# Hengle/AkariRender-1

Measured on AMD Instinct MI355X. Metric: Msamples/sec (whole node), 10M-tri scene 1080p 1024spp, 1/2/4/8 MI355X, higher is better.
Workload: dtype f32; 1 GPU; C3 synthetic triangle soup (SURVEY.md §8d); triangles=10000002, width=1920, height=1080, spp=1025, max_depth=5, tile=64, parallelism=tile-split x1, bvh_leaf=4, builder=sbvh, form=k_path, ordered_fetch=True

## Files before the change

akarirender-1_amd/csrc/capi.hip:

```cpp
#include <hip/hip_runtime.h>

#include <algorithm>
#include <atomic>
#include <chrono>
#include <cmath>
#include <cstring>
#include <map>
#include <memory>
#include <stdexcept>
#include <string>
#include <thread>
#include <vector>

#include "akr_device.h"
#include "bvh_build.h"
#include "kernels.h"
#include "options.h"
#include "path_plan.h"

using namespace akr;

#define HIPCHK(x)                                                                                        \
    do {                                                                                                 \
        hipError_t e_ = (x);                                                                             \
        if (e_ != hipSuccess) throw std::runtime_error(std::string(#x) + " failed: " + hipGetErrorString(e_)); \
    } while (0)

namespace {

template <class T>
struct DBuf {
    T *p = nullptr;
    size_t n = 0;
    DBuf() = default;
    DBuf(const DBuf &) = delete;
    DBuf &operator=(const DBuf &) = delete;
    ~DBuf() { release(); }
    void release() {
        if (p) (void)hipFree(p);
        p = nullptr;
        n = 0;
    }
    void reserve(size_t count) {
        if (count <= n && p) return;
        release();
        size_t c = std::max<size_t>(count, 1);
        HIPCHK(hipMalloc(reinterpret_cast<void **>(&p), c * sizeof(T)));
        n = c;
    }
    void upload(const T *h, size_t count, hipStream_t st) {
// ... 91 lines not shown
    std::string err;
    Options opt;
    hipEvent_t ev_done = nullptr;
    bool done_recorded = false;
    DBuf<uint32_t> d_bad;
    uint32_t *h_check = nullptr, *d_check_host = nullptr;
    uint32_t *h_fault = nullptr, *d_fault_host = nullptr;
    DBuf<uint4> d_probe;
    uint64_t probe_n = 0;
    bool probe_ok = false;

    std::vector<float> verts;
    std::vector<int32_t> idx;
    std::vector<float> normals, texcoords;
    std::vector<int32_t> matid;
    std::vector<uint32_t> mesh_base{0};
    std::vector<akr_texture> texs;
    std::vector<akr_material> mats;
    std::vector<float> images;
    std::vector<int64_t> img_off;
    std::vector<int32_t> img_w, img_h;
    std::vector<akr_area_light> lights;
    std::vector<float> power;
    bool scene_dirty = true;
    bool accel_built = false;
    akr_accel_info info{};
    BvhOutput bvh;
    Bvh4Output bvh4;

    DBuf<akr_bvh_node> d_nodes;
    DBuf<akr_bvh4_node> d_wnodes;
    DBuf<float4> d_wleaves;
    uint32_t wide_root_dev = AKR_CHILD_EMPTY;
    uint64_t bvh_dev_bytes = 0;
    DBuf<float4> d_tris;
    DBuf<ShadeTri> d_shade_tri;
    DBuf<float> d_tc, d_images, d_cdf, d_func;
    DBuf<MatDev> d_mats;
    DBuf<TexDev> d_texs;
    DBuf<LightDev> d_lights;
    DBuf<uint32_t> d_mesh_base;
    float func_int = 0;
    int32_t n_lights = 0;
    int32_t n_mats = 0;
    bool has_image_tex = false;
    bool simple_shading = true;

    CameraDev cam{};
    bool cam_set = false;

    EnvDev env{};
    DBuf<float4> d_env_map;
    DBuf<float> d_env_tab;
    bool env_on() const { return env.n > 0; }
    const EnvDev &require_env() const {
        if (!env_on()) throw std::runtime_error("no environment light (akr_hip_upload_environment)");
        return env;
    }

    size_t cap = 0;
    std::vector<uint4> h_tiles;
    uint64_t n_pix_last = 0;
    DBuf<uint4> d_tiles;
    struct Session {
        bool valid = false, seeded = false;
        uint64_t n = 0;
// ... 494 lines not shown
        HIPCHK(hipMemsetAsync(d_owork.p, 0, kTraceWords * sizeof(uint32_t), ms));
        const uint32_t sub = (uint32_t)opt.path_order_sub, n_rays = (uint32_t)(((uint64_t)N + (1u << sub) - 1) >> sub);
        launch_pilot_rays(cam, d_pixel.p, n_rays, sub, d_ray0.p, ms);
        TraceArgs t = trace_args(d_owork.p);
        t.rays = d_ray0.p;
        t.n = n_rays;
        t.hits = d_hit.p;
        t.counters = d_ocnt.p;
        t.ray_steps = d_okey[1].p;
        t.step_cap = (uint32_t)opt.path_order_cap;
        launch_trace(TRACE_PILOT, false, true, true, t, grid_for(TRACE_CLOSEST, n_rays), ms);
        if (sum_steps) HIPCHK(hipMemsetAsync(d_steps_sum.p, 0, sizeof(unsigned long long), ms));
        launch_order_keys(d_okey[1].p, N, (uint32_t)opt.path_order_shift, (uint32_t)(opt.path_order_classes - 1), sub,
                          d_okey[0].p, d_oidx[0].p, ms, sum_steps ? d_steps_sum.p : nullptr);
        sort_pixel_order(d_otmp.p, tb, d_okey[0].p, d_okey[1].p, d_oidx[0].p, d_oidx[1].p, N, ms);
        HIPCHK(hipGetLastError());
    }

    void probe_render(const PathArgs &base, bool tab, uint32_t N, int S, hipStream_t ms) {
        if (d_pprobe.n < N) throw std::runtime_error("pilot probe buffer not sized");
        HIPCHK(hipMemsetAsync(d_owork.p, 0, kTraceWords * sizeof(uint32_t), ms));
        PathArgs pp = base;
        pp.spp = (uint32_t)S;
        pp.work = d_owork.p;
        pp.t.counters = d_ocnt.p;
        pp.prof = nullptr;
        pp.probe = d_pprobe.p;
        pp.probe_clock = 0;
        pp.order = nullptr;
        pp.fault_test = 0;
        pp.state_in = pp.state_out = nullptr;
        const uint32_t grid = (uint32_t)std::max<uint64_t>(
            1, std::min<uint64_t>(path_grid[PATH_PLAIN][tab], ((uint64_t)N + kTraceBlock - 1) / kTraceBlock));
        launch_path(true, PATH_PLAIN, tab, pp, grid, ms);
        HIPCHK(hipMemsetAsync(d_film.p, 0, (size_t)N * sizeof(float4), ms));
    }

    void resolve_form() {
        if (!form_pending && !pilot_sum_pending) return;
        if (done_recorded) HIPCHK(hipStreamWaitEvent(stream, ev_done, 0));
        unsigned long long sum = 0;
        uint32_t gate = 0;
        HIPCHK(hipMemcpyAsync(&sum, d_steps_sum.p, sizeof(sum), hipMemcpyDeviceToHost, stream));
        if (form_pending) HIPCHK(hipMemcpyAsync(&gate, d_gate.p, sizeof(gate), hipMemcpyDeviceToHost, stream));
        HIPCHK(hipStreamSynchronize(stream));
        last_pilot_steps = (int64_t)sum;
        if (form_pending) {
            if (gate > 1) throw std::runtime_error("render form gate holds " + std::to_string(gate));
            last_form = gate_forms[gate];
        }
        form_pending = pilot_sum_pending = false;
    }

    void pixel_order_path(const PathArgs &base, bool tab, uint32_t N, int S, hipStream_t ms) {
        if (d_okey[0].n < N || d_oidx[0].n < N) throw std::runtime_error("pixel order buffers not sized");
        const uint32_t max_rays = (uint32_t)S * (2u * (uint32_t)std::max(base.max_depth, 0) + 1u);
        probe_render(base, tab, N, S, ms);
        launch_probe_cost(d_pprobe.p, N, d_okey[1].p, ms);
        uint32_t shift = 0;
        while (((max_rays + 1u) >> shift) > (uint32_t)opt.path_order_classes) shift++;
        launch_order_keys(d_okey[1].p, N, shift, (uint32_t)(opt.path_order_classes - 1), 0, d_okey[0].p, d_oidx[0].p, ms);
        sort_pixel_order(d_otmp.p, d_otmp.n, d_okey[0].p, d_okey[1].p, d_oidx[0].p, d_oidx[1].p, N, ms);
        HIPCHK(hipGetLastError());
    }

    uint64_t setup_pixels(const akr_rect *tiles, int32_t n_tiles, size_t n_count_words, hipStream_t st) {
        require_ready();
// ... 332 lines not shown
        for (int k = 0; k < 3; k++) in.grid[k] = path_grid[k][tab];
        in.block = kTraceBlock;
        const PathPlan pl = plan_path(in, opt);
        last_ppl1000 = pl.ppl1000;
        last_pilot_rays = pl.pilot_rays;
        last_pilot_steps = -1;
        if (opt.path_order != 0) warm_order(N, ms);
        if (pl.pilot) {
            if (pl.path_pilot)
                timed("pilot", ms, [&] { pixel_order_path(pa, tab, (uint32_t)N, opt.path_order_pilot_spp, ms); });
            else
                timed("pilot", ms, [&] { pixel_order((uint32_t)N, ms, pl.want_steps); });
        }
        if (pl.gated)
            launch_pick_form(d_steps_sum.p, (unsigned long long)opt.path_tail_steps * (uint64_t)pl.pilot_rays, d_gate.p, ms);
        PathArgs args[2] = {pa, pa};
        for (int k = 0; k < pl.n_launch; k++) {
            const PathLaunch &l = pl.launch[k];
            PathArgs &x = args[k];
            if (l.contrib_lanes) {
                d_contrib.reserve((size_t)18 * l.contrib_lanes);
                x.contrib = d_contrib.p;
            }
            x.mix = l.mix;
            x.order = l.list == LIST_PILOT ? d_oidx[1].p : (l.list == LIST_SUBSET ? r.subset : nullptr);
            x.order_mode = l.order_mode;
            x.prio = l.prio;
            if (pl.gated) {
                x.gate = d_gate.p;
                x.gate_want = (uint32_t)k;
            }
        }
        timed("path", ms, [&] {
            for (int k = 0; k < pl.n_launch; k++) launch_path(opt.count, pl.launch[k].kind, tab, args[k], pl.launch[k].grid, ms);
        });
        HIPCHK(hipGetLastError());
        form_pending = pl.gated;
        pilot_sum_pending = pl.want_steps && !pl.gated;
        if (pl.gated) std::copy(pl.gate_forms, pl.gate_forms + 2, gate_forms);
        last_form = pl.last_form;
        last_ordered = pl.last_ordered;
        if (r.subset && r.probe)
            launch_probe_fill(d_seed.p, (uint32_t)N, r.probe, AKR_PROBE_SEED | (opt.count ? AKR_PROBE_RAYS : 0u), ms);
    }

    void render_wavefront(const Pass &r) {
        const akr_pt_params &p = r.p;
        const uint64_t N = r.N, M = r.M;
        const uint32_t *subset = r.subset;
        const bool resume = r.resume, tight = r.tight;
        uint4 *probe_p = r.probe;
        const size_t n_count_words = r.n_count_words;
        const int D = p.max_depth + 2;
        hipStream_t ms = main_st;
        const SceneDev sd = scene_dev();
        if (p.spp > 0) last_form = AKR_FORM_WAVEFRONT;
        const int nb = p.max_depth == 0 ? 1 : p.max_depth;
        int64_t g = 0;
        const uint32_t *worder = nullptr;
        if (opt.wave_order && opt.path_order != 0 && !subset && p.spp >= order_min_spp(opt, N) && N >= 2) {
            warm_order(N, ms);
            timed("pilot", ms, [&] { pixel_order((uint32_t)N, ms); });
            worder = d_oidx[1].p;
        }
        last_ordered = worder ? 1 : 0;
        for (int s = 0; s < p.spp; s++) {
            const int ps = s & 1;
// ... 589 lines not shown
                want[3 + k] = v1[k] - v0[k];
                want[6 + k] = v2[k] - v0[k];
            }
            const float got[9] = {tr[r].v0[0], tr[r].v0[1], tr[r].v0[2], tr[r].e1[0], tr[r].e1[1],
                                  tr[r].e1[2], tr[r].e2[0], tr[r].e2[1], tr[r].e2[2]};
            if (std::memcmp(want, got, sizeof(want)) != 0) {
                bad[t] = r;
                return;
            }
            covered[g].store(1, std::memory_order_relaxed);
        }
    });
    for (uint64_t r : bad)
        if (r != UINT64_MAX)
            throw std::runtime_error("imported BVH: triangle record " + std::to_string(r) + " (gid " +
                                     std::to_string(tr[r].gid) + ") does not match this scene's triangle");
    for (uint64_t g = 0; g < nt; g++)
        if (!covered[g].load(std::memory_order_relaxed))
            throw std::runtime_error("imported BVH: scene triangle " + std::to_string(g) + " is in no leaf");
}

void finish_accel(akr_hip_ctx *ctx, int n_threads) {
        auto &b = ctx->bvh;
        ctx->accel_built = false;
        {
            Bvh4Output w;
            build_bvh4(b.nodes, w, n_threads, ctx->wide_collapse);
            if (w.nodes.size() >= kMaxWideNodes)
                throw std::runtime_error("scene too large: the wide view needs fewer than 2^26 nodes (about 100 M triangles)");
            ctx->bvh4 = std::move(w);
        }
        ctx->d_nodes.upload(b.nodes.data(), b.nodes.size(), ctx->stream);
        const auto &leaves = ctx->bvh4.leaves;
        std::vector<uint32_t> leaf_off(leaves.size());
        size_t words = 0;
        const size_t align = (size_t)std::max(1, ctx->opt.leaf_align);
        for (size_t i = 0; i < leaves.size(); i++) {
            words = (words + align - 1) / align * align;
            if (words >= AKR_CHILD_LEAF) break;
            leaf_off[i] = (uint32_t)words;
            words += 2 + 3 * (size_t)leaves[i].count;
        }
        if (words >= AKR_CHILD_LEAF) throw std::runtime_error("BVH too large for the wide leaf blob");
        const size_t pad = 3;
        std::unique_ptr<float4[]> blob(new float4[words + pad]);
        if (align > 1) std::memset(static_cast<void *>(blob.get()), 0, sizeof(float4) * (words + pad));
        else std::memset(static_cast<void *>(blob.get() + words), 0, sizeof(float4) * pad);
        const float4 *tri4 = reinterpret_cast<const float4 *>(b.tris.data());
        std::vector<akr_bvh4_node> wn = ctx->bvh4.nodes;
        auto remap = [&](uint32_t r) {
            return (r != AKR_CHILD_EMPTY && (r & AKR_CHILD_LEAF)) ? (AKR_CHILD_LEAF | leaf_off[r & 0x7FFFFFFFu]) : r;
        };
        const int nt = n_threads > 0 ? std::min(n_threads, 64)
                                       : (int)std::min(64u, std::max(1u, std::thread::hardware_concurrency()));
        auto fill = [&](int t) {
            const size_t l0 = leaves.size() * t / nt, l1 = leaves.size() * (t + 1) / nt;
            for (size_t i = l0; i < l1; i++) {
                const akr_bvh_leaf &l = leaves[i];
                float4 *o = blob.get() + leaf_off[i];
                float4 h0, h1;
                h0.x = l.lo[0], h0.y = l.lo[1], h0.z = l.lo[2], h0.w = l.hi[0];
                uint32_t fc[2] = {l.first, l.count};
                h1.x = l.hi[1], h1.y = l.hi[2];
                std::memcpy(&h1.z, &fc[0], 4);
                std::memcpy(&h1.w, &fc[1], 4);
                o[0] = h0;
                o[1] = h1;
                std::memcpy(o + 2, tri4 + 3 * (size_t)l.first, sizeof(float4) * 3 * (size_t)l.count);
            }
            const size_t n0 = wn.size() * t / nt, n1 = wn.size() * (t + 1) / nt;
            for (size_t i = n0; i < n1; i++)
                for (auto &c : wn[i].child) c = remap(c);
        };
        run_on_threads(nt, fill);
        ctx->wide_root_dev = remap(ctx->bvh4.root_ref);
        ctx->d_wnodes.reserve(1);
        ctx->d_wleaves.reserve(1);
        ctx->d_wnodes.upload(wn.data(), wn.size(), ctx->stream);
        ctx->d_wleaves.upload(blob.get(), words + pad, ctx->stream);
        ctx->bvh_dev_bytes = (uint64_t)wn.size() * sizeof(akr_bvh4_node) + (uint64_t)(words + pad) * sizeof(float4);
        HIPCHK(hipStreamSynchronize(ctx->stream));
        ctx->d_tris.upload(reinterpret_cast<const float4 *>(b.tris.data()), 3 * b.tris.size(), ctx->stream);
        HIPCHK(hipStreamSynchronize(ctx->stream));
        ctx->info.n_nodes = b.nodes.size();
        ctx->info.n_tris = b.tris.size();
        ctx->info.max_depth = b.max_depth;
        ctx->info.max_leaf = b.max_leaf;
        ctx->info.build_ms = b.build_ms;
        ctx->info.sah_cost = b.sah_cost;
        ctx->accel_built = true;
        ctx->commit_scene();
}
}

int akr_hip_build_accel(akr_hip_ctx *ctx, const akr_build_params *params) {
    return guard(ctx, [&] {
        akr_build_params p{};
        p.max_leaf_size = 4;
        p.n_bins = 32;
        p.traversal_cost = 1.0f;
        p.intersect_cost = 4.0f;
        if (params) p = *params;
        BvhInput in{ctx->verts.data(), ctx->idx.data(), ctx->n_tris()};
        ctx->drop_session();
        ctx->accel_built = false;
        if (p.builder == AKR_BUILDER_LBVH) build_lbvh_gpu(in, ctx->bvh, ctx->stream);
        else if (p.builder == AKR_BUILDER_SAH || p.builder == AKR_BUILDER_SBVH) build_bvh(in, p, ctx->bvh);
        else throw std::runtime_error("unknown builder");
// ... 1047 lines not shown
```

akarirender-1_amd/csrc/kernels.h:

```cpp
#pragma once
#include "akr_device.h"

namespace akr {

enum : int { TRACE_CLOSEST = 0, TRACE_ANY = 1, TRACE_SHADOW = 2, TRACE_PILOT = 3 };

void launch_trace(int mode, bool count, bool tight, bool wide, const TraceArgs &a, uint32_t grid, hipStream_t st);
int trace_blocks_per_cu(int mode);
void launch_raygen(const RaygenArgs &a, hipStream_t st);
void launch_shade(const ShadeArgs &a, uint32_t max_items, hipStream_t st);
void launch_splat(const SplatArgs &a, uint32_t max_items, hipStream_t st);
void launch_shade_env(const ShadeEnvArgs &a, uint32_t max_items, hipStream_t st);
void launch_shade_mis(const ShadeMisArgs &a, uint32_t max_items, hipStream_t st);
void launch_shade_env_mis(const ShadeEnvMisArgs &a, uint32_t max_items, hipStream_t st);
void launch_splat_mis(const SplatMisArgs &a, uint32_t max_items, hipStream_t st);
void launch_env_unit(bool sample, const EnvUnitArgs &a, hipStream_t st);
void launch_pick_form(const unsigned long long *sum, unsigned long long thresh, uint32_t *gate, hipStream_t st);
void launch_store_word(const uint32_t *src, uint32_t *dst, hipStream_t st);
void launch_ao_shade(const AoShadeArgs &a, uint32_t max_items, hipStream_t st);
void launch_ao_resolve(const AoResolveArgs &a, uint32_t max_items, hipStream_t st);
void launch_path(bool count, int kind, bool tab, const PathArgs &a, uint32_t grid, hipStream_t st);
int path_blocks_per_cu(int kind, bool tab);
bool path_tab_fits(int32_t n_mats, int32_t n_lights);
void launch_check_weights(const float4 *film, uint32_t n, float expect, uint32_t *bad, hipStream_t st);
void launch_merge_film(const float4 *film, const uint32_t *pixel, const uint32_t *order, uint32_t n, int32_t width,
                       float *rad, float *w, hipStream_t st);
void launch_unpack(const float4 *film, uint32_t n, float *rad, float *w, hipStream_t st);
void launch_expand_pixels(const uint4 *tiles, uint32_t n_tiles, uint32_t n, uint32_t *pixel, hipStream_t st);
void launch_probe_seed(const uint32_t *seed, uint32_t n, uint4 *probe, hipStream_t st);
void launch_probe_cost(const uint4 *probe, uint32_t n, uint32_t *cost, hipStream_t st);
constexpr uint32_t kOrderClassBits = 5, kOrderClassMask = (1u << kOrderClassBits) - 1u;
void launch_pilot_rays(const CameraDev &cam, const uint32_t *pixel, uint32_t n, uint32_t sub, float4 *rays,
                       hipStream_t st);
void launch_order_keys(const uint32_t *steps, uint32_t n, uint32_t shift, uint32_t cmax, uint32_t sub, uint32_t *key,
                       uint32_t *idx, hipStream_t st, unsigned long long *sum = nullptr);
size_t pixel_order_tmp_bytes(uint32_t n);
void sort_pixel_order(void *tmp, size_t tmp_bytes, const uint32_t *key_in, uint32_t *key_out, const uint32_t *idx_in,
                      uint32_t *idx_out, uint32_t n, hipStream_t st);

void launch_mask_count(const uint8_t *mask, uint32_t n, uint32_t *wcount, hipStream_t st);
size_t scan_tmp_bytes(uint32_t n);
void scan_exclusive_u32(void *tmp, size_t tmp_bytes, const uint32_t *in, uint32_t *out, uint32_t n, hipStream_t st);
void launch_mask_compact(const uint8_t *mask, uint32_t n, const uint32_t *woff, uint32_t *list, uint32_t *total,
                         hipStream_t st);
void launch_fill_u32(uint32_t *p, uint32_t n, uint32_t v, hipStream_t st);
void launch_count_add(uint32_t *count, const uint32_t *list, uint32_t n, uint32_t spp, hipStream_t st);
void launch_check_counts(const float4 *film, const uint32_t *count, uint32_t n, uint32_t *bad, hipStream_t st);
void launch_count_range(const uint32_t *count, const uint32_t *list, uint32_t n, uint32_t *out, hipStream_t st);
void launch_init_seed(const uint32_t *pixel, uint32_t n, int32_t width, uint32_t *seed, hipStream_t st);
void launch_probe_fill(const uint32_t *seed, uint32_t n, uint4 *probe, uint32_t flags, hipStream_t st);
void launch_adaptive_test(const float4 *film, float4 *prev, uint32_t n, float threshold, float *strip_err,
                          uint8_t *strip_active, uint8_t *mask, hipStream_t st);

void launch_feature_rays(const CameraDev &cam, const uint32_t *pixel, uint32_t n, uint32_t *seed, bool first,
// ... 31 lines not shown
```

akarirender-1_amd/csrc/kernels.hip:

```cpp
#include "akr_device.h"
#include "akr_math.h"
#include "kernels.h"

namespace akr {

__device__ __forceinline__ uint32_t fbits(float f) { return __float_as_uint(f); }
__device__ __forceinline__ float bitsf(uint32_t u) { return __uint_as_float(u); }

template <bool TIGHT, bool FAST = false>
__device__ __forceinline__ float box_test(float lox, float hix, float loy, float hiy, float loz, float hiz, V3 o,
                                          V3 invd, float tmin, float tmax) {
    float t0x = (lox - o.x) * invd.x, t1x = (hix - o.x) * invd.x;
    float t0y = (loy - o.y) * invd.y, t1y = (hiy - o.y) * invd.y;
    float t0z = (loz - o.z) * invd.z, t1z = (hiz - o.z) * invd.z;
    float m0, m1, t;
    if (FAST) {
        m0 = fmaxf(fmaxf(fminf(t0x, t1x), fminf(t0y, t1y)), fminf(t0z, t1z));
        m1 = fminf(fminf(fmaxf(t0x, t1x), fmaxf(t0y, t1y)), fmaxf(t0z, t1z));
        t = fmaxf(tmin, m0);
    } else {
        m0 = rmax(rmax(rmin(t0x, t1x), rmin(t0y, t1y)), rmin(t0z, t1z));
        m1 = rmin(rmin(rmax(t0x, t1x), rmax(t0y, t1y)), rmax(t0z, t1z));
        t = rmax(tmin, m0);
    }
    bool hit = m0 <= m1 && !(t >= tmax);
    if (TIGHT) hit = hit && t <= m1;
    return hit ? t : -1.0f;
}

__device__ __forceinline__ bool fast_box_ok(V3 o, V3 invd, float tmin, float tmax) {
    return isfinite(o.x) && isfinite(o.y) && isfinite(o.z) && isfinite(invd.x) && isfinite(invd.y) &&
           isfinite(invd.z) && invd.x != 0.0f && invd.y != 0.0f && invd.z != 0.0f && !isnan(tmin) && !isnan(tmax);
}

__device__ __forceinline__ bool mt(V3 o, V3 d, float tmin, float tmax, float4 a, float4 b, float4 c, float best,
// ... 503 lines not shown
                        deep = deep || sp > kStackLds;
                    }
                    if (STEPS && a.step_cap && steps >= a.step_cap) cur = AKR_CHILD_EMPTY;
                } else if (!WIDE && busy && is_internal(cur)) {
                    if (COUNT) {
                        c_box += 2;
                        c_visit++;
                    }
                    if (wave_fast)
                        visit_node<TIGHT, true, ANY>(nodesf, nodesu, cur, o, d, invd, tmin, tmax, best, s_stack,
                                                     stack_ovf, a.ovf_threads, tid, gtid, sp);
                    else
                        visit_node<TIGHT, false, ANY>(nodesf, nodesu, cur, o, d, invd, tmin, tmax, best, s_stack,
                                                      stack_ovf, a.ovf_threads, tid, gtid, sp);
                    if (COUNT) deep = deep || sp > kStackLds;
                }
                if (busy && !need_pop && leaf == AKR_CHILD_EMPTY && is_leaf(cur)) {
                    leaf = cur;
                    need_pop = true;
                }
                if (need_pop)
                    cur = stack_pop(s_stack, stack_ovf, a.ovf_threads, tid, gtid, sp, ANY ? (kOnePop ? tmaxp : tmax) : best);
                const unsigned long long searching = __ballot(busy && leaf == AKR_CHILD_EMPTY && cur != AKR_CHILD_EMPTY);
                if ((uint32_t)__popcll(searching) <= (uint32_t)(ANY ? kWhileExitAny : kWhileExit) &&
                    (searching == 0 || __ballot(busy && leaf != AKR_CHILD_EMPTY) != 0))
                    break;
            }
            if (busy && leaf != AKR_CHILD_EMPTY) {
                uint32_t cnt;
                const float4 *tp;
                float4 pa, pb, pc;
                float4 pa1, pb1, pc1;
                if (WIDE) {
                    const float4 *lr = a.wide_leaves + (leaf & 0x7FFFFFFFu);
                    const float4 l0 = lr[0], l1 = lr[1];
                    pa = lr[2];
                    pb = lr[3];
                    pc = lr[4];
                    pa1 = lr[5];
                    pb1 = lr[6];
                    pc1 = lr[7];
                    issue_together(pa, pb, pc, pa1, pb1, pc1);
                    const float tl = box_test<TIGHT, true>(l0.x, l0.w, l0.y, l1.x, l0.z, l1.y, o, invd, tmin, tmax);
                    const bool in = !(tl < 0.0f || tl > (ANY ? tmax : best));
                    if (COUNT) {
                        c_box++;
                        c_leaf++;
                    }
                    cnt = in ? fbits(l1.w) : 0u;
                    tp = lr + 2;
                } else {
                    tp = a.tris + 3 * (size_t)akr_leaf_first(leaf);
                    cnt = akr_leaf_count(leaf);
                    pa = tp[0];
                    pb = tp[1];
                    pc = tp[2];
                }
                for (uint32_t k = 0; k < cnt; k++) {
                    if (COUNT && lane_prefix(__ballot(1)) == 0) c_stri += 64;
                    const float4 ta = k == 0 ? pa : (WIDE && k == 1 ? pa1 : tp[3 * k + 0]);
                    const float4 tb = k == 0 ? pb : (WIDE && k == 1 ? pb1 : tp[3 * k + 1]);
                    const float4 tc = k == 0 ? pc : (WIDE && k == 1 ? pc1 : tp[3 * k + 2]);
                    if (COUNT) c_tri++;
                    if (STEPS) steps++;
                    float t, u, v;
                    if (mt(o, d, tmin, tmax, ta, tb, tc, ANY ? kInf : best, t, u, v)) {
                        best = t;
// ... 955 lines not shown
    }
    const uint32_t cnt = in ? fbits(l1.w) : 0u;
    const float4 *tp = lr + 2;
    for (uint32_t k = 0; k < cnt; k++) {
        if (COUNT && lane_prefix(__ballot(1)) == 0) c.stri += 64;
        const float4 ta = k == 0 ? pa0 : (k == 1 ? pa1 : tp[3 * k + 0]);
        const float4 tb = k == 0 ? pb0 : (k == 1 ? pb1 : tp[3 * k + 1]);
        const float4 tc = k == 0 ? pc0 : (k == 1 ? pc1 : tp[3 * k + 2]);
        if (COUNT) {
            c.tri[kind]++;
            if (c.lines && k >= 2) mark_lines(c.lines, c.span[1], c.span[2], c.leaf_base, tp + 3 * k, 48u);
        }
        float t, u, v;
        if (mt(r.o, r.d, r.tmin, r.tmax, ta, tb, tc, r.best, t, u, v)) {
            r.best = t;
            r.bu = u;
            r.bv = v;
            r.bgid = fbits(ta.w);
            if (kind) {
                hit_any = true;
                break;
            }
        }
    }
    r.leaf = AKR_CHILD_EMPTY;
    return hit_any;
}

template <bool COUNT>
__device__ __forceinline__ bool path_leaf(bool busy, int kind, PathRay &r, const float4 *wide_leaves, PathCount &c) {
    if constexpr (!COUNT) {
        bool hit_any = false;
        if (busy && r.leaf != AKR_CHILD_EMPTY) {
            const float4 *lr = wide_leaves + (r.leaf & 0x7FFFFFFFu);
            const float4 l0 = lr[0], l1 = lr[1];
            const float4 pa0 = lr[2], pb0 = lr[3], pc0 = lr[4];
            const float4 pa1 = lr[5], pb1 = lr[6], pc1 = lr[7];
            issue_together(pa0, pb0, pc0, pa1, pb1, pc1);
            const float tl = box_test<true, true>(l0.x, l0.w, l0.y, l1.x, l0.z, l1.y, r.o, r.invd, r.tmin, r.tmax);
            const bool in = !(tl < 0.0f || tl > r.best);
            const uint32_t cnt = in ? fbits(l1.w) : 0u;
            const float4 *tp = lr + 2;
            for (uint32_t k = 0; k < cnt; k++) {
                const float4 ta = k == 0 ? pa0 : (k == 1 ? pa1 : tp[3 * k + 0]);
                const float4 tb = k == 0 ? pb0 : (k == 1 ? pb1 : tp[3 * k + 1]);
                const float4 tc = k == 0 ? pc0 : (k == 1 ? pc1 : tp[3 * k + 2]);
                float t, u, v;
                if (mt(r.o, r.d, r.tmin, r.tmax, ta, tb, tc, r.best, t, u, v)) {
                    r.best = t;
                    r.bu = u;
                    r.bv = v;
                    r.bgid = fbits(ta.w);
                    if (kind) {
                        hit_any = true;
                        break;
                    }
                }
            }
            r.leaf = AKR_CHILD_EMPTY;
        }
        return hit_any;
    } else {
        bool hit_any = false;
        const unsigned long long ta = wall_clock64();
        const bool in_leaf = busy && r.leaf != AKR_CHILD_EMPTY;
        const uint32_t holders = (uint32_t)__popcll(__ballot(in_leaf));
        c.lphases += holders ? 1u : 0u;
        c.lholders += holders;
        const float4 *lr = wide_leaves + (in_leaf ? (r.leaf & 0x7FFFFFFFu) : 0u);
        const float4 l0 = lr[0], l1 = lr[1], pa0 = lr[2], pb0 = lr[3], pc0 = lr[4], pa1 = lr[5], pb1 = lr[6],
                     pc1 = lr[7];
        const unsigned long long tb = wall_clock64();
        asm volatile("s_waitcnt vmcnt(0)" ::: "memory");
        const unsigned long long tc = wall_clock64();
        if (in_leaf && c.lines) mark_lines(c.lines, c.span[1], c.span[2], wide_leaves, lr, 128u);
        if (in_leaf) hit_any = leaf_tests<true>(kind, r, lr, l0, l1, pa0, pb0, pc0, pa1, pb1, pc1, c);
        c.tl_issue += tb - ta;
        c.tl_wait += tc - tb;
        c.tl_comp += wall_clock64() - tc;
        return hit_any;
    }
}

template <bool COUNT>
__device__ __forceinline__ bool path_begin(const TraceArgs &a, bool occl, float4 ra, float4 rb, PathRay &r,
                                           lds_u64 *s_stack, glb_u64 *ovf, uint32_t tid, uint32_t gtid, PathCount &c) {
    r.o = V3{ra.x, ra.y, ra.z};
    r.d = V3{rb.x, rb.y, rb.z};
    r.tmin = ra.w;
    r.tmax = rb.w;
    r.invd = V3{1.0f / r.d.x, 1.0f / r.d.y, 1.0f / r.d.z};
    r.dpos = (r.d.x > 0.0f ? 1u : 0u) | (r.d.y > 0.0f ? 2u : 0u) | (r.d.z > 0.0f ? 4u : 0u);
    if (occl && a.any_far_first) r.dpos ^= 7u;
    r.tmaxp = float_below(r.tmax);
    if (COUNT) c.rays[occl]++;
    if (!lean_ok(r.o, r.invd, r.tmin, r.tmax)) {
        bool hit;
        if (occl)
            trace_exact_core<true, true>(a, r.o, r.d, r.invd, r.tmin, r.tmax, s_stack, ovf, tid, gtid, r.best, r.bu,
                                         r.bv, r.bgid, hit);
        else
            trace_exact_core<false, true>(a, r.o, r.d, r.invd, r.tmin, r.tmax, s_stack, ovf, tid, gtid, r.best, r.bu,
                                          r.bv, r.bgid, hit);
        return false;
    }
    r.best = occl ? r.tmax : kInf;
    r.bu = r.bv = 0.0f;
    r.bgid = kNoHit;
    r.sp = 0;
    r.leaf = AKR_CHILD_EMPTY;
    if (COUNT) {
        c.box[occl]++;
        c.deep_now = false;
    }
// ... 119 lines not shown
    }
    const int slot_of[2] = {TRACE_CLOSEST, TRACE_SHADOW};
    for (int m = 0; m < 2; m++) {
        const unsigned long long rr = wave_sum(c.rays[m]), b = wave_sum(c.box[m]), t = wave_sum(c.tri[m]),
                                 v = wave_sum(c.visit[m]), dp = wave_sum(c.deep[m]), lf = wave_sum(c.leaf[m]);
        if (__lane_id() == 0) {
            TraceCounters &tc = a.counters[slot_of[m]];
            atomicAdd(&tc.rays, rr);
            atomicAdd(&tc.box, b);
            atomicAdd(&tc.tri, t);
            atomicAdd(&tc.visits, v);
            atomicAdd(&tc.deep, dp);
            atomicAdd(&tc.leaves, lf);
        }
    }
    const unsigned long long st = wave_sum(c.strav), sl = wave_sum(c.sleaf), sr = wave_sum(c.stri);
    if (__lane_id() == 0) {
        atomicAdd(&a.counters[TRACE_CLOSEST].slots_trav, st);
        atomicAdd(&a.counters[TRACE_CLOSEST].slots_leaf, sl);
        atomicAdd(&a.counters[TRACE_CLOSEST].slots_tri, sr);
    }
}

template <bool COUNT>
__device__ __forceinline__ uint32_t probe_flags(const PathArgs &pa) {
    if (!COUNT) return AKR_PROBE_SEED;
    uint32_t f = AKR_PROBE_SEED | AKR_PROBE_RAYS;
    if (pa.probe_clock) f |= 4u | (uint32_t)((wall_clock64() >> 4) << 8);
    return f;
}

constexpr int kParkSlots = 8;

template <bool COUNT, bool TAB>
__global__ __launch_bounds__(kTraceBlock) __attribute__((amdgpu_waves_per_eu(AKR_PATH_WAVES))) void k_path(PathArgs pa) {
    if (pa.gate && *pa.gate != pa.gate_want) return;
    const TraceArgs &a = pa.t;
    __shared__ unsigned long long s_stack_mem[kStackLdsU64];
    __shared__ uint32_t s_park[kParkSlots][kTraceBlock];
    __shared__ uint4 s_tab[TAB ? kTabBytes / 16 : 1];
    lds_u64 *s_stack = (lds_u64 *)s_stack_mem;
    glb_u64 *stack_ovf = (glb_u64 *)a.stack_ovf;
    const uint32_t tid = threadIdx.x;
    const uint32_t gtid = blockIdx.x * kTraceBlock + tid;
    const uint32_t n = pa.n_pix;
    const int nb = pa.max_depth == 0 ? 1 : pa.max_depth;
    const bool ff = a.any_far_first != 0;
    const auto tab = PathTab<TAB>::make(pa.sc, s_tab);
    static_assert(kParkSlots >= 1 && kTraceBlock % 64 == 0, "the push's scratch words lie in a wave's park row 0");
    lds_u64 *dead = (lds_u64 *)&s_park[0][0] + (tid >> 1);
    PathCount c;
    if (COUNT) {
        c.lines = pa.lines;
        c.span[1] = pa.lines_span[1];
        c.span[2] = pa.lines_span[2];
        c.leaf_base = a.wide_leaves;
    }
    PixelFetch f{blockIdx.x % kWorkShards, 0, 0, (int)kWorkShards, n == 0};
    f.s_lo = shard_begin(n, f.shard);
    f.s_hi = shard_begin(n, f.shard + 1);

    uint32_t pix = 0, left = 0, seed = 0, pxr = 0;
    int depth = 0;
    V3 beta{1.0f, 1.0f, 1.0f}, Lr{0.0f, 0.0f, 0.0f}, scol{0.0f, 0.0f, 0.0f};
    float4 film = {0.0f, 0.0f, 0.0f, 0.0f};
    float4 pe0 = {}, pe1 = {};
    enum : uint32_t { F_BUSY = 1u, F_DONE = 2u, F_FIN = 4u, F_NEED = 8u, F_ANY = 16u, F_PEND = 32u };
    uint32_t fl = F_NEED;
// ... 129 lines not shown
                const uint32_t px = pxr;
                camera_ray(pa.cam, (int)(px & 0xFFFFu), (int)(px >> 16), seed, ra, rb);
                fresh = true;
            }
            asm volatile("" ::: "memory");
            if (COUNT) {
                const unsigned long long t = wall_clock64();
                p_tnext += t - p_ts;
                p_ts = t;
            }
            path_unpark(s_park, tid, r, ff, any);
            if (fresh) {
                any = next_any;
                if (COUNT) {
                    pc_closest += any ? 0u : 1u;
                    pc_shadow += any ? 1u : 0u;
                }
                busy = path_begin<COUNT>(a, any, ra, rb, r, s_stack, stack_ovf, tid, gtid, c);
                fin = !busy;
            }
            fl = (busy ? F_BUSY : 0u) | (done ? F_DONE : 0u) | (fin ? F_FIN : 0u) | (need_pixel ? F_NEED : 0u) |
                 (any ? F_ANY : 0u) | (pend ? F_PEND : 0u);
            asm("" : "+v"(fl));
            if (COUNT) p_tbegin += wall_clock64() - p_ts;
        }
        if (COUNT) {
            const unsigned long long t = wall_clock64();
            p_tp += t - p_t;
            p_t = t;
        }
        const unsigned long long bm = mask_of((fl & F_BUSY) != 0);
        if (bm == 0) continue;
        const bool busy = in_mask(bm);
        const int kd = (fl & F_ANY) != 0 ? 1 : 0;
        if constexpr (COUNT)
            path_traverse<COUNT, kWhileExitPath, true>(busy, kd, r, a.wide_nodes, s_stack, stack_ovf, a.ovf_threads, tid,
                                                       gtid, c, pa.pop_keep, pa.pop_rounds, dead);
        else
            path_traverse_masks<kWhileExitPath>(bm, r, a.wide_nodes, s_stack, stack_ovf, a.ovf_threads, tid, gtid,
                                                pa.pop_keep, pa.pop_rounds, dead);
        if (COUNT) {
            const unsigned long long t = wall_clock64();
            p_tt += t - p_t;
            p_t = t;
        }
        const bool hit_any = path_leaf<COUNT>(busy, kd, r, a.wide_leaves, c);
        const bool ended = busy && (hit_any || r.cur == AKR_CHILD_EMPTY);
        fl = ended ? (fl ^ (F_BUSY | F_FIN)) : fl;
        if (COUNT && ended) c.deep[kd] += c.deep_now ? 1 : 0;
        if (COUNT) p_tl += wall_clock64() - p_t;
    }
    if (COUNT) {
        path_count_flush(pa, c, p_outer, p_procs, p_tp, p_tt, p_tl, p_t0, p_lanes, p_tsh);
        if (__lane_id() == 0 && pa.prof) {
            atomicAdd(&pa.prof->tp_park, p_tpark);
            atomicAdd(&pa.prof->tp_next, p_tnext);
            atomicAdd(&pa.prof->tp_begin, p_tbegin);
            atomicAdd(&pa.prof->tp_load, p_tload);
        }
    }
}

__device__ __forceinline__ void path_park(uint32_t (*s_park)[kTraceBlock], uint32_t tid, const PathRay &r) {
    const float pv[8] = {r.o.x, r.o.y, r.o.z, r.d.x, r.d.y, r.d.z, r.tmin, r.tmax};
#pragma unroll
    for (int k = 0; k < 8; k++) s_park[k][tid] = fbits(pv[k]);
}
__device__ __forceinline__ void path_unpark(uint32_t (*s_park)[kTraceBlock], uint32_t tid, PathRay &r, bool far_first,
                                            bool occl) {
    r.o = V3{bitsf(s_park[0][tid]), bitsf(s_park[1][tid]), bitsf(s_park[2][tid])};
    r.d = V3{bitsf(s_park[3][tid]), bitsf(s_park[4][tid]), bitsf(s_park[5][tid])};
    r.tmin = bitsf(s_park[6][tid]);
    r.tmax = bitsf(s_park[7][tid]);
    r.invd = V3{1.0f / r.d.x, 1.0f / r.d.y, 1.0f / r.d.z};
    r.dpos = (r.d.x > 0.0f ? 1u : 0u) | (r.d.y > 0.0f ? 2u : 0u) | (r.d.z > 0.0f ? 4u : 0u);
    if (occl && far_first) r.dpos ^= 7u;
    r.tmaxp = float_below(r.tmax);
    r.leaf = AKR_CHILD_EMPTY;
}

__device__ __forceinline__ int nth_set_bit(unsigned long long m, uint32_t r) {
    int base = 0;
#pragma unroll
    for (int s = 32; s > 0; s >>= 1) {
        const unsigned long long low = m & ((1ull << s) - 1ull);
        const uint32_t c = (uint32_t)__popcll(low);
        if (r >= c) {
            r -= c;
            m >>= s;
            base += s;
        } else {
            m = low;
        }
// ... 1073 lines not shown
void launch_pick_form(const unsigned long long *sum, unsigned long long thresh, uint32_t *gate, hipStream_t st) {
    hipLaunchKernelGGL(k_pick_form, dim3(1), dim3(64), 0, st, sum, thresh, gate);
}
void launch_store_word(const uint32_t *src, uint32_t *dst, hipStream_t st) {
    hipLaunchKernelGGL(k_store_word, dim3(1), dim3(64), 0, st, src, dst);
}
void launch_shade_mis(const ShadeMisArgs &a, uint32_t max_items, hipStream_t st) {
    if (max_items == 0) return;
    const dim3 grid((uint32_t)((max_items + kShadeBlock - 1) / kShadeBlock));
    hipLaunchKernelGGL(k_shade_mis, grid, dim3(kShadeBlock), 0, st, a);
}
void launch_shade_env_mis(const ShadeEnvMisArgs &a, uint32_t max_items, hipStream_t st) {
    if (max_items == 0) return;
    const dim3 grid((uint32_t)((max_items + kShadeBlock - 1) / kShadeBlock));
    hipLaunchKernelGGL(k_shade_env_mis, grid, dim3(kShadeBlock), 0, st, a);
}
void launch_ao_shade(const AoShadeArgs &a, uint32_t max_items, hipStream_t st) {
    if (max_items == 0) return;
    hipLaunchKernelGGL(k_ao_shade, dim3(blocks_for(max_items)), dim3(kBlock), 0, st, a);
}
void launch_ao_resolve(const AoResolveArgs &a, uint32_t max_items, hipStream_t st) {
    if (max_items == 0) return;
    hipLaunchKernelGGL(k_ao_resolve, dim3(blocks_for(max_items)), dim3(kBlock), 0, st, a);
}
void launch_splat(const SplatArgs &a, uint32_t max_items, hipStream_t st) {
    if (max_items == 0) return;
    hipLaunchKernelGGL(k_splat, dim3(blocks_for(max_items)), dim3(kBlock), 0, st, a);
}
void launch_splat_mis(const SplatMisArgs &a, uint32_t max_items, hipStream_t st) {
    if (max_items == 0) return;
    hipLaunchKernelGGL(k_splat_mis, dim3(blocks_for(max_items)), dim3(kBlock), 0, st, a);
}
using PathKernel = void (*)(PathArgs);
static PathKernel path_kernel(int kind, bool count, bool tab) {
    if (count && tab) {
        if (kind == PATH_DEFER) return k_path_defer<true, true>;
        if (kind == PATH_SPEC) return k_path_spec<true, true>;
        return k_path<true, true>;
    }
    if (count) {
        if (kind == PATH_DEFER) return k_path_defer<true, false>;
        if (kind == PATH_SPEC) return k_path_spec<true, false>;
        return k_path<true, false>;
    }
    if (kind == PATH_SPEC) return tab ? k_path_spec<false, true> : k_path_spec<false, false>;
    if (kind == PATH_DEFER) return tab ? k_path_defer<false, true> : k_path_defer<false, false>;
    return tab ? k_path<false, true> : k_path<false, false>;
}
void launch_path(bool count, int kind, bool tab, const PathArgs &a, uint32_t grid, hipStream_t st) {
    if (grid == 0) return;
    if (tab && !path_tab_fits(a.sc.n_mats, a.sc.n_lights)) tab = false;
    hipLaunchKernelGGL(path_kernel(kind, count, tab), dim3(grid), dim3(kTraceBlock), 0, st, a);
}
int path_blocks_per_cu(int kind, bool tab) {
    int nb = 0;
    const hipError_t e = hipOccupancyMaxActiveBlocksPerMultiprocessor(&nb, path_kernel(kind, false, tab), kTraceBlock, 0);
    if (e != hipSuccess || nb <= 0) nb = 1;
    return nb;
}
void launch_check_weights(const float4 *film, uint32_t n, float expect, uint32_t *bad, hipStream_t st) {
    if (n == 0) return;
    hipLaunchKernelGGL(k_check_weights, dim3(blocks_for(n)), dim3(kBlock), 0, st, film, n, expect, bad);
}
void launch_merge_film(const float4 *film, const uint32_t *pixel, const uint32_t *order, uint32_t n, int32_t width,
                       float *rad, float *w, hipStream_t st) {
    if (n == 0) return;
    hipLaunchKernelGGL(k_merge_film, dim3(blocks_for(n)), dim3(kBlock), 0, st, film, pixel, order, n, width, rad, w);
}
void launch_pilot_rays(const CameraDev &cam, const uint32_t *pixel, uint32_t n, uint32_t sub, float4 *rays,
                       hipStream_t st) {
    if (n == 0) return;
    hipLaunchKernelGGL(k_pilot_rays, dim3(blocks_for(n)), dim3(kBlock), 0, st, cam, pixel, n, sub, rays);
}
void launch_order_keys(const uint32_t *steps, uint32_t n, uint32_t shift, uint32_t cmax, uint32_t sub, uint32_t *key,
                       uint32_t *idx, hipStream_t st, unsigned long long *sum) {
    if (n == 0) return;
    hipLaunchKernelGGL(k_order_keys, dim3(blocks_for(n)), dim3(kBlock), 0, st, steps, n, shift,
                       cmax < kOrderClassMask ? cmax : kOrderClassMask, sub, key, idx, sum);
}
void launch_probe_cost(const uint4 *probe, uint32_t n, uint32_t *cost, hipStream_t st) {
    if (n) hipLaunchKernelGGL(k_probe_cost, dim3(blocks_for(n)), dim3(kBlock), 0, st, probe, n, cost);
}
void launch_probe_seed(const uint32_t *seed, uint32_t n, uint4 *probe, hipStream_t st) {
    if (n == 0) return;
    hipLaunchKernelGGL(k_probe_seed, dim3(blocks_for(n)), dim3(kBlock), 0, st, seed, n, probe);
// ... 49 lines not shown
```

Baseline: 569.6 Msamples/s.

## Tag single-triangle leaves and use a lean one-triangle leaf path in k_path

```diff
diff --git a/akarirender-1_amd/csrc/capi.hip b/akarirender-1_amd/csrc/capi.hip
--- a/akarirender-1_amd/csrc/capi.hip
+++ b/akarirender-1_amd/csrc/capi.hip
@@ -16,6 +16,7 @@
 #include "bvh_build.h"
 #include "kernels.h"
 #include "options.h"
+#include "leaf_layout.h"
 #include "path_plan.h"
 
 using namespace akr;
@@ -173,6 +174,7 @@
     DBuf<akr_bvh4_node> d_wnodes;
     DBuf<float4> d_wleaves;
     uint32_t wide_root_dev = AKR_CHILD_EMPTY;
+    bool leaf_one_kernel = false;
     uint64_t bvh_dev_bytes = 0;
     DBuf<float4> d_tris;
     DBuf<ShadeTri> d_shade_tri;
@@ -733,7 +735,7 @@
         pp.state_in = pp.state_out = nullptr;
         const uint32_t grid = (uint32_t)std::max<uint64_t>(
             1, std::min<uint64_t>(path_grid[PATH_PLAIN][tab], ((uint64_t)N + kTraceBlock - 1) / kTraceBlock));
-        launch_path(true, PATH_PLAIN, tab, pp, grid, ms);
+        launch_path(true, PATH_PLAIN, tab, leaf_one_kernel, pp, grid, ms);
         HIPCHK(hipMemsetAsync(d_film.p, 0, (size_t)N * sizeof(float4), ms));
     }
 
@@ -1132,7 +1134,7 @@
             }
         }
         timed("path", ms, [&] {
-            for (int k = 0; k < pl.n_launch; k++) launch_path(opt.count, pl.launch[k].kind, tab, args[k], pl.launch[k].grid, ms);
+            for (int k = 0; k < pl.n_launch; k++) launch_path(opt.count, pl.launch[k].kind, tab, leaf_one_kernel, args[k], pl.launch[k].grid, ms);
         });
         HIPCHK(hipGetLastError());
         form_pending = pl.gated;
@@ -1788,24 +1790,19 @@
         }
         ctx->d_nodes.upload(b.nodes.data(), b.nodes.size(), ctx->stream);
         const auto &leaves = ctx->bvh4.leaves;
-        std::vector<uint32_t> leaf_off(leaves.size());
-        size_t words = 0;
-        const size_t align = (size_t)std::max(1, ctx->opt.leaf_align);
-        for (size_t i = 0; i < leaves.size(); i++) {
-            words = (words + align - 1) / align * align;
-            if (words >= AKR_CHILD_LEAF) break;
-            leaf_off[i] = (uint32_t)words;
-            words += 2 + 3 * (size_t)leaves[i].count;
-        }
-        if (words >= AKR_CHILD_LEAF) throw std::runtime_error("BVH too large for the wide leaf blob");
-        const size_t pad = 3;
+        const akr::LeafLayout lay = akr::leaf_layout(leaves.size(), (size_t)std::max(1, ctx->opt.leaf_align),
+                                                     [&](size_t i) { return leaves[i].count; });
+        const std::vector<uint32_t> &leaf_off = lay.offset;
+        const size_t words = lay.words, pad = akr::kLeafBlobPad, align = (size_t)std::max(1, ctx->opt.leaf_align);
         std::unique_ptr<float4[]> blob(new float4[words + pad]);
         if (align > 1) std::memset(static_cast<void *>(blob.get()), 0, sizeof(float4) * (words + pad));
         else std::memset(static_cast<void *>(blob.get() + words), 0, sizeof(float4) * pad);
         const float4 *tri4 = reinterpret_cast<const float4 *>(b.tris.data());
         std::vector<akr_bvh4_node> wn = ctx->bvh4.nodes;
         auto remap = [&](uint32_t r) {
-            return (r != AKR_CHILD_EMPTY && (r & AKR_CHILD_LEAF)) ? (AKR_CHILD_LEAF | leaf_off[r & 0x7FFFFFFFu]) : r;
+            if (r == AKR_CHILD_EMPTY || !(r & AKR_CHILD_LEAF)) return r;
+            const uint32_t i = r & 0x7FFFFFFFu;
+            return lay.ref(i, leaves[i].count);
         };
         const int nt = n_threads > 0 ? std::min(n_threads, 64)
                                        : (int)std::min(64u, std::max(1u, std::thread::hardware_concurrency()));
@@ -1830,6 +1827,9 @@
         };
         run_on_threads(nt, fill);
         ctx->wide_root_dev = remap(ctx->bvh4.root_ref);
+        size_t n_one = 0;
+        for (const akr_bvh_leaf &l : leaves) n_one += l.count == 1 ? 1 : 0;
+        ctx->leaf_one_kernel = akr::leaf_one_pays(n_one, leaves.size());
         ctx->d_wnodes.reserve(1);
         ctx->d_wleaves.reserve(1);
         ctx->d_wnodes.upload(wn.data(), wn.size(), ctx->stream);
diff --git a/akarirender-1_amd/csrc/kernels.h b/akarirender-1_amd/csrc/kernels.h
--- a/akarirender-1_amd/csrc/kernels.h
+++ b/akarirender-1_amd/csrc/kernels.h
@@ -19,7 +19,7 @@
 void launch_store_word(const uint32_t *src, uint32_t *dst, hipStream_t st);
 void launch_ao_shade(const AoShadeArgs &a, uint32_t max_items, hipStream_t st);
 void launch_ao_resolve(const AoResolveArgs &a, uint32_t max_items, hipStream_t st);
-void launch_path(bool count, int kind, bool tab, const PathArgs &a, uint32_t grid, hipStream_t st);
+void launch_path(bool count, int kind, bool tab, bool leaf_one, const PathArgs &a, uint32_t grid, hipStream_t st);
 int path_blocks_per_cu(int kind, bool tab);
 bool path_tab_fits(int32_t n_mats, int32_t n_lights);
 void launch_check_weights(const float4 *film, uint32_t n, float expect, uint32_t *bad, hipStream_t st);
diff --git a/akarirender-1_amd/csrc/kernels.hip b/akarirender-1_amd/csrc/kernels.hip
--- a/akarirender-1_amd/csrc/kernels.hip
+++ b/akarirender-1_amd/csrc/kernels.hip
@@ -1,6 +1,7 @@
 #include "akr_device.h"
 #include "akr_math.h"
 #include "kernels.h"
+#include "leaf_layout.h"
 
 namespace akr {
 
@@ -570,7 +571,7 @@
                 float4 pa, pb, pc;
                 float4 pa1, pb1, pc1;
                 if (WIDE) {
-                    const float4 *lr = a.wide_leaves + (leaf & 0x7FFFFFFFu);
+                    const float4 *lr = a.wide_leaves + (leaf & kLeafOffsetMask);
                     const float4 l0 = lr[0], l1 = lr[1];
                     pa = lr[2];
                     pb = lr[3];
@@ -1592,7 +1593,7 @@
     if constexpr (!COUNT) {
         bool hit_any = false;
         if (busy && r.leaf != AKR_CHILD_EMPTY) {
-            const float4 *lr = wide_leaves + (r.leaf & 0x7FFFFFFFu);
+            const float4 *lr = wide_leaves + (r.leaf & kLeafOffsetMask);
             const float4 l0 = lr[0], l1 = lr[1];
             const float4 pa0 = lr[2], pb0 = lr[3], pc0 = lr[4];
             const float4 pa1 = lr[5], pb1 = lr[6], pc1 = lr[7];
@@ -1627,7 +1628,7 @@
         const uint32_t holders = (uint32_t)__popcll(__ballot(in_leaf));
         c.lphases += holders ? 1u : 0u;
         c.lholders += holders;
-        const float4 *lr = wide_leaves + (in_leaf ? (r.leaf & 0x7FFFFFFFu) : 0u);
+        const float4 *lr = wide_leaves + (in_leaf ? (r.leaf & kLeafOffsetMask) : 0u);
         const float4 l0 = lr[0], l1 = lr[1], pa0 = lr[2], pb0 = lr[3], pc0 = lr[4], pa1 = lr[5], pb1 = lr[6],
                      pc1 = lr[7];
         const unsigned long long tb = wall_clock64();
@@ -1640,6 +1641,47 @@
         c.tl_comp += wall_clock64() - tc;
         return hit_any;
     }
+}
+
+__device__ __forceinline__ unsigned long long path_leaf_masks(unsigned long long bm, unsigned long long am, PathRay &r,
+                                                              const float4 *wide_leaves) {
+    const unsigned long long hold = bm & mask_of(r.leaf != AKR_CHILD_EMPTY);
+    const unsigned long long one = hold & mask_of((r.leaf & kLeafOne) != 0);
+    unsigned long long hm = 0;
+    const bool several = hold != one;
+    if (__builtin_expect(one != 0 && !several, 1)) {
+        const float4 *lr = wide_leaves + (in_mask(one) ? (r.leaf & kLeafOffsetMask) : 0u);
+        const float4 l0 = lr[0], l1 = lr[1];
+        const float4 a = lr[2], b = lr[3], c = lr[4];
+        const float tl = box_test<true, true>(l0.x, l0.w, l0.y, l1.x, l0.z, l1.y, r.o, r.invd, r.tmin, r.tmax);
+        const unsigned long long out = mask_of(tl < 0.0f) | mask_of(tl > r.best);
+        const V3 v0{a.x, a.y, a.z}, e1{b.x, b.y, b.z}, e2{c.x, c.y, c.z};
+        const V3 h = cross(r.d, e2);
+        const float det = dot(e1, h);
+        const unsigned long long flat = mask_of(det > -1e-6f) & mask_of(det < 1e-6f);
+        const float f = 1.0f / det;
+        const V3 s = sub(r.o, v0);
+        const float u = f * dot(s, h);
+        const unsigned long long out_u = mask_of(u < 0.0f) | mask_of(u > 1.0f);
+        const V3 q = cross(s, e1);
+        const float v = f * dot(r.d, q);
+        const unsigned long long out_v = mask_of(v < 0.0f) | mask_of(u + v > 1.0f);
+        const float t = f * dot(e2, q);
+        const unsigned long long near = mask_of(t > r.tmin) & mask_of(t < r.tmax) & mask_of(t < r.best);
+        const unsigned long long hit = one & near & ~(out | flat | out_u | out_v);
+        const bool won = in_mask(hit);
+        r.best = won ? t : r.best;
+        r.bu = won ? u : r.bu;
+        r.bv = won ? v : r.bv;
+        r.bgid = won ? fbits(a.w) : r.bgid;
+        r.leaf = in_mask(one) ? AKR_CHILD_EMPTY : r.leaf;
+        hm = hit & am;
+    }
+    if (__builtin_expect(several, 0)) {
+        PathCount none{};
+        hm |= mask_of(path_leaf<false>(in_mask(bm), in_mask(am) ? 1 : 0, r, wide_leaves, none));
+    }
+    return hm;
 }
 
 template <bool COUNT>
@@ -1825,8 +1867,8 @@
 
 constexpr int kParkSlots = 8;
 
-template <bool COUNT, bool TAB>
-__global__ __launch_bounds__(kTraceBlock) __attribute__((amdgpu_waves_per_eu(AKR_PATH_WAVES))) void k_path(PathArgs pa) {
+template <bool COUNT, bool TAB, bool ONE>
+__device__ __forceinline__ void path_plain(const PathArgs &pa) {
     if (pa.gate && *pa.gate != pa.gate_want) return;
     const TraceArgs &a = pa.t;
     __shared__ unsigned long long s_stack_mem[kStackLdsU64];
@@ -2022,7 +2064,7 @@
         const unsigned long long bm = mask_of((fl & F_BUSY) != 0);
         if (bm == 0) continue;
         const bool busy = in_mask(bm);
-        const int kd = (fl & F_ANY) != 0 ? 1 : 0;
+        [[maybe_unused]] const int kd = (fl & F_ANY) != 0 ? 1 : 0;
         if constexpr (COUNT)
             path_traverse<COUNT, kWhileExitPath, true>(busy, kd, r, a.wide_nodes, s_stack, stack_ovf, a.ovf_threads, tid,
                                                        gtid, c, pa.pop_keep, pa.pop_rounds, dead);
@@ -2034,8 +2076,14 @@
             p_tt += t - p_t;
             p_t = t;
         }
-        const bool hit_any = path_leaf<COUNT>(busy, kd, r, a.wide_leaves, c);
-        const bool ended = busy && (hit_any || r.cur == AKR_CHILD_EMPTY);
+        bool ended;
+        if constexpr (COUNT || !ONE) {
+            const bool hit_any = path_leaf<COUNT>(busy, kd, r, a.wide_leaves, c);
+            ended = busy && (hit_any || r.cur == AKR_CHILD_EMPTY);
+        } else {
+            const unsigned long long hm = path_leaf_masks(bm, mask_of((fl & F_ANY) != 0), r, a.wide_leaves);
+            ended = in_mask(bm & (hm | mask_of(r.cur == AKR_CHILD_EMPTY)));
+        }
         fl = ended ? (fl ^ (F_BUSY | F_FIN)) : fl;
         if (COUNT && ended) c.deep[kd] += c.deep_now ? 1 : 0;
         if (COUNT) p_tl += wall_clock64() - p_t;
@@ -2049,6 +2097,15 @@
             atomicAdd(&pa.prof->tp_load, p_tload);
         }
     }
+}
+
+template <bool COUNT, bool TAB>
+__global__ __launch_bounds__(kTraceBlock) __attribute__((amdgpu_waves_per_eu(AKR_PATH_WAVES))) void k_path(PathArgs pa) {
+    path_plain<COUNT, TAB, true>(pa);
+}
+template <bool TAB>
+__global__ __launch_bounds__(kTraceBlock) __attribute__((amdgpu_waves_per_eu(AKR_PATH_WAVES))) void k_path_general(PathArgs pa) {
+    path_plain<false, TAB, false>(pa);
 }
 
 __device__ __forceinline__ void path_park(uint32_t (*s_park)[kTraceBlock], uint32_t tid, const PathRay &r) {
@@ -3188,7 +3245,7 @@
     hipLaunchKernelGGL(k_splat_mis, dim3(blocks_for(max_items)), dim3(kBlock), 0, st, a);
 }
 using PathKernel = void (*)(PathArgs);
-static PathKernel path_kernel(int kind, bool count, bool tab) {
+static PathKernel path_kernel(int kind, bool count, bool tab, bool leaf_one = true) {
     if (count && tab) {
         if (kind == PATH_DEFER) return k_path_defer<true, true>;
         if (kind == PATH_SPEC) return k_path_spec<true, true>;
@@ -3201,12 +3258,13 @@
     }
     if (kind == PATH_SPEC) return tab ? k_path_spec<false, true> : k_path_spec<false, false>;
     if (kind == PATH_DEFER) return tab ? k_path_defer<false, true> : k_path_defer<false, false>;
+    if (!leaf_one) return tab ? k_path_general<true> : k_path_general<false>;
     return tab ? k_path<false, true> : k_path<false, false>;
 }
-void launch_path(bool count, int kind, bool tab, const PathArgs &a, uint32_t grid, hipStream_t st) {
+void launch_path(bool count, int kind, bool tab, bool leaf_one, const PathArgs &a, uint32_t grid, hipStream_t st) {
     if (grid == 0) return;
     if (tab && !path_tab_fits(a.sc.n_mats, a.sc.n_lights)) tab = false;
-    hipLaunchKernelGGL(path_kernel(kind, count, tab), dim3(grid), dim3(kTraceBlock), 0, st, a);
+    hipLaunchKernelGGL(path_kernel(kind, count, tab, leaf_one), dim3(grid), dim3(kTraceBlock), 0, st, a);
 }
 int path_blocks_per_cu(int kind, bool tab) {
     int nb = 0;
diff --git a/akarirender-1_amd/csrc/leaf_layout.h b/akarirender-1_amd/csrc/leaf_layout.h
--- /dev/null
+++ b/akarirender-1_amd/csrc/leaf_layout.h
@@ -0,0 +1,43 @@
+#pragma once
+#include <stddef.h>
+#include <stdint.h>
+
+#include <stdexcept>
+#include <vector>
+
+#include "../../include/akr_bvh_format.h"
+
+namespace akr {
+
+constexpr uint32_t kLeafOne = 1u << 30;
+constexpr uint32_t kLeafOffsetMask = kLeafOne - 1u;
+constexpr size_t kLeafBlobPad = 3;
+
+inline bool leaf_one_pays(size_t n_one, size_t n_leaves) { return n_leaves > 0 && n_one * 100 >= n_leaves * 97; }
+
+struct LeafLayout {
+    std::vector<uint32_t> offset;
+    size_t words = 0;
+
+    uint32_t ref(size_t i, uint32_t count) const { return AKR_CHILD_LEAF | (count == 1 ? kLeafOne : 0u) | offset[i]; }
+};
+
+template <class Count>
+inline LeafLayout leaf_layout(size_t n_leaves, size_t align, Count count) {
+    LeafLayout l;
+    l.offset.resize(n_leaves);
+    if (align < 1) align = 1;
+    size_t words = 0;
+    for (size_t i = 0; i < n_leaves && words < kLeafOne; i++) {
+        words = (words + align - 1) / align * align;
+        if (words >= kLeafOne) break;
+        l.offset[i] = (uint32_t)words;
+        words += 2 + 3 * (size_t)count(i);
+    }
+    if (words >= kLeafOne)
+        throw std::runtime_error("BVH too large for the wide leaf blob: a leaf reference holds a 30-bit float4 offset (16 GB)");
+    l.words = words;
+    return l;
+}
+
+}
```

New measurement: 583.8 Msamples/s (median of 6 runs). 1.02x the previous value.
